# facebookresearch/theseus

Hardware: NVIDIA H100
Metric: LM iterations/sec on batched SE3 pose-graph (2500 poses, global batch 2048 over N GPUs, LM + block-sparse Cholesky, fp64) (higher is better)
Workload: dtype f64

## Files before the change

### theseus_b200/csrc/thb_front.cu

```cuda
#include <stdlib.h>

#include "thb_common.cuh"

namespace thb {

__device__ __forceinline__ void record_first_failure(int* info, int pos) {
  int old = 0;
  while (true) {
    const int prev = atomicCAS(info, old, pos);
    if (prev == old || (prev != 0 && prev <= pos)) return;
    old = prev;
  }
}

#ifdef THB_SIMT_EMU
#define THB_PDL_TRIGGER() do { } while (0)
#define THB_PDL_WAIT() do { } while (0)
#define FRONT_LAUNCH(K, grid, block, smem, cs, arg) K<<<grid, block, smem, cs>>>(arg)
#else
#define THB_PDL_TRIGGER() asm volatile("griddepcontrol.launch_dependents;" ::: "memory")
#define THB_PDL_WAIT() asm volatile("griddepcontrol.wait;" ::: "memory")
#define FRONT_LAUNCH(K, grid, block, smem, cs, arg) thb::front_launch_pdl(K, grid, block, smem, cs, arg)
static inline bool front_pdl_enabled() {
  static const bool on = [] { const char* e = getenv("THB_FRONT_PDL"); return e != nullptr && e[0] == '1'; }();
  return on;
}
template <typename A>
static inline void front_launch_pdl(void (*kernel)(A), dim3 grid, dim3 block, size_t smem, cudaStream_t cs, const A& arg) {
  cudaLaunchConfig_t cfg = {};
  cfg.gridDim = grid; cfg.blockDim = block; cfg.dynamicSmemBytes = smem; cfg.stream = cs;
  cudaLaunchAttribute at[1];
  at[0].id = cudaLaunchAttributeProgrammaticStreamSerialization;
  at[0].val.programmaticStreamSerializationAllowed = 1;
  cfg.attrs = at; cfg.numAttrs = front_pdl_enabled() ? 1 : 0;
  cudaLaunchKernelEx(&cfg, kernel, arg);
}
#endif

#ifdef THB_SIMT_EMU
__device__ inline void front_mma884(double& c0, double& c1, double a, double b) {
  const int lane = threadIdx.x & 31, lr = lane >> 2, lc = lane & 3;
  for (int k = 0; k < 4; k++) {
    const double av = __shfl_sync(0xffffffffu, a, lr * 4 + k);
    const double b0 = __shfl_sync(0xffffffffu, b, (2 * lc) * 4 + k);
    const double b1 = __shfl_sync(0xffffffffu, b, (2 * lc + 1) * 4 + k);
    c0 += av * b0;
    c1 += av * b1;
  }
}
#else
__device__ __forceinline__ void front_mma884(double& c0, double& c1, double a, double b) {
  asm volatile("mma.sync.aligned.m8n8k4.row.col.f64.f64.f64.f64 {%0,%1}, {%2}, {%3}, {%0,%1};\n" : "+d"(c0), "+d"(c1) : "d"(a), "d"(b));
}
#endif

__host__ __device__ __forceinline__ int front_pad_ld(int x) { return ((x + 11) / 16) * 16 + 4; }

struct FrontArgs {
  thb_front_plan p;
  int s0;
  int64_t B;
  double* factor;
  const double* alpha;
  const double* beta;
  double* arena_cur;
  const double* arena_child;
  int32_t* info;
  int prefetch;
  const double* ata;
  int64_t ata_stride;
  const double* rhs;
  double* work;
  double* v_cur;
  const double* v_child;
};

__device__ __forceinline__ double front_panel_in(const FrontArgs& a, const double* Lg, int64_t poff, int64_t item, int64_t e) {
  if (a.ata == nullptr) return Lg[e];
  const int32_t m = a.p.pmap[poff + e];
  return m >= 0 ? a.ata[item * a.ata_stride + m] : 0.0;
}

template <typename T>
__device__ __forceinline__ T front_ldg(const T* p) {
#ifdef THB_SIMT_EMU
  return *p;
#else
  return __ldg(p);
#endif
}


constexpr int FRONT_WD_LD = 20;
#ifndef FRONT_PL
#define FRONT_PL 4
#endif
constexpr int FRONT_MAX_CHILDREN = 8;

__host__ __device__ __forceinline__ int64_t front_smem_doubles(int w, int b, int nchildren) {
  const int b16 = (b + 15) & ~15, w8 = (w + 7) & ~7;
  return (int64_t)(w8 + b16 + 8) * front_pad_ld(w8) + 8 * FRONT_WD_LD + 3 * FRONT_MAX_CHILDREN
         + ((int64_t)nchildren * (w + b) + 1) / 2 + 2;
}

__device__ __forceinline__ int front_leaf8(double* __restrict__ T, int ld, double* __restrict__ Wd, int lane) {
  const int ln = lane < 8 ? lane : 0;
  double row[8];
#pragma unroll
  for (int q = 0; q < 8; q++) row[q] = T[ln * ld + q];
  int fail = 0;
  double invd = 0.0;
#pragma unroll
  for (int c = 0; c < 8; c++) {
    const double d = __shfl_sync(0xffffffffu, row[c], c);
    if (!(d > 0.0) && fail == 0) fail = c + 1;
    double inv = rsqrt(d);
    inv = inv * (1.5 - 0.5 * d * inv * inv);
    const double sq = d * inv;
    if (lane == c) invd = inv;
    const double lrc = (lane == c) ? sq : row[c] * inv;
    row[c] = lrc;
#pragma unroll
    for (int q = c + 1; q < 8; q++) {
      const double lqc = __shfl_sync(0xffffffffu, lrc, q);
      row[q] -= lrc * lqc;
    }
  }
  if (lane < 8) {
#pragma unroll
    for (int q = 0; q < 8; q++)
      if (q <= lane) T[lane * ld + q] = row[q];
  }
  double x[8];
#pragma unroll
  for (int rr = 0; rr < 8; rr++) {
    double sacc = (lane == rr) ? 1.0 : 0.0;
#pragma unroll
    for (int k = 0; k < rr; k++) {
      const double lrk = __shfl_sync(0xffffffffu, row[k], rr);
      sacc -= lrk * x[k];
    }
    x[rr] = sacc * __shfl_sync(0xffffffffu, invd, rr);
  }
  if (lane < 8) {
#pragma unroll
    for (int rr = 0; rr < 8; rr++) Wd[rr * FRONT_WD_LD + lane] = (rr >= lane) ? x[rr] : 0.0;
  }
  return fail;
}

__device__ __forceinline__ void front_diag_block(double* PN, int ldp, int jb, double* Wd, int lane, int w, int first, int32_t* info) {
  const int lr = lane >> 2, lc = lane & 3;
  double c0 = 0.0, c1 = 0.0;
  const double* Arow = PN + (8 * jb + lr) * ldp + lc;
  for (int k = 0; k < 8 * jb; k += 4) {
    const double av = Arow[k];
    front_mma884(c0, c1, av, av);
  }
  double* d = PN + (8 * jb + lr) * ldp + 8 * jb + 2 * lc;
  d[0] -= c0;
  d[1] -= c1;
  __syncwarp();
  const int fail = front_leaf8(PN + (8 * jb) * ldp + 8 * jb, ldp, Wd, lane);
  if (lane == 0 && fail != 0 && 8 * jb + fail <= w) record_first_failure(info, first + 8 * jb + fail);
}

template <bool TWO>
__device__ __forceinline__ void front_tile_column(double* PN, int ldp, int jb, int rt0, const double* Wd, int lane) {
  const int lr = lane >> 2, lc = lane & 3;
  double x00 = 0.0, x01 = 0.0, x10 = 0.0, x11 = 0.0;
  const double* A0 = PN + (8 * rt0 + lr) * ldp + lc;
  const double* Bj = PN + (8 * jb + lr) * ldp + lc;
  for (int k = 0; k < 8 * jb; k += 4) {
    const double bf = Bj[k];
    front_mma884(x00, x01, A0[k], bf);
    if (TWO) front_mma884(x10, x11, A0[8 * ldp + k], bf);
  }
  double* X0 = PN + (8 * rt0 + lr) * ldp + 8 * jb + 2 * lc;
  X0[0] -= x00; X0[1] -= x01;
  if (TWO) { X0[8 * ldp] -= x10; X0[8 * ldp + 1] -= x11; }
  __syncwarp();
  x00 = x01 = x10 = x11 = 0.0;
#pragma unroll
  for (int k = 0; k < 8; k += 4) {
    const double bf = Wd[lr * FRONT_WD_LD + k + lc];
    front_mma884(x00, x01, A0[8 * jb + k], bf);
    if (TWO) front_mma884(x10, x11, A0[8 * ldp + 8 * jb + k], bf);
  }
  __syncwarp();
  X0[0] = x00; X0[1] = x01;
  if (TWO) { X0[8 * ldp] = x10; X0[8 * ldp + 1] = x11; }
}

struct FrontChild {
  const double* src;
  int ldg, lo, hi, uoff;
};

__device__ __forceinline__ void front_panel_gather2(const FrontChild* ch, const int32_t* INV, int r, int nch, int q, const int* ii,
                                                    const int* jj, double (&x)[2][FRONT_PL]) {
#pragma unroll
  for (int c = 0; c < 2; c++) {
    int lo = r, hi = -1, ldg = 0;
    const double* src = nullptr;
    if (q + c < nch) { lo = ch[q + c].lo; hi = ch[q + c].hi; ldg = ch[q + c].ldg; src = ch[q + c].src; }
    const int32_t* inv = INV + (q + c) * r;
#pragma unroll
    for (int u = 0; u < FRONT_PL; u++) {
      x[c][u] = -0.0;
      if (ii[u] >= lo && jj[u] <= hi) {
        const int ci = inv[ii[u]], cj = inv[jj[u]];
        if (ci >= 0 && cj >= 0) x[c][u] = front_ldg(src + (int64_t)ci * ldg + cj);
      }
    }
  }
}

__device__ __forceinline__ int front_next_child(unsigned& mask) {
#ifdef THB_SIMT_EMU
  const int q = __builtin_ctz(mask);
#else
  const int q = __ffs(mask) - 1;
#endif
  mask &= mask - 1;
  return q;
}

__device__ __forceinline__ void front_tile_gather(const FrontChild& c, const int32_t* inv, int r, int li0, int lj0, double (&x)[2][2][2]) {
  int ci[2], cj[2][2];
#pragma unroll
  for (int mi = 0; mi < 2; mi++) ci[mi] = (li0 + 8 * mi < r) ? inv[li0 + 8 * mi] : -1;
#pragma unroll
  for (int ni = 0; ni < 2; ni++)
#pragma unroll
    for (int u = 0; u < 2; u++) cj[ni][u] = (lj0 + 8 * ni + u < r) ? inv[lj0 + 8 * ni + u] : -1;
#pragma unroll
  for (int mi = 0; mi < 2; mi++)
#pragma unroll
    for (int ni = 0; ni < 2; ni++)
#pragma unroll
      for (int u = 0; u < 2; u++)
        x[mi][ni][u] = (ci[mi] >= 0 && cj[ni][u] >= 0 && cj[ni][u] <= ci[mi]) ? front_ldg(c.src + (int64_t)ci[mi] * c.ldg + cj[ni][u]) : -0.0;
}

__device__ __forceinline__ double front_warp_trsv_lower(const double* T, int ld, double ui, int cw, int lane) {
  const double rd = lane < cw ? 1.0 / T[lane * ld + lane] : 0.0;
  for (int k = 0; k < cw; k++) {
    const double yk = __shfl_sync(0xffffffffu, ui * rd, k);
    if (lane == k) ui = yk;
    else if (lane > k && lane < cw) ui -= T[lane * ld + k] * yk;
  }
  return ui;
}

struct FrontRowsGlobal {
  static constexpr bool kInPanel = false;
  const double* L;
  int w;
  double* T;
  __device__ __forceinline__ const double* row(int i) const { return L + (int64_t)i * w; }
  __device__ __forceinline__ const double* diag(int k0, int cw, int tid, int nthreads, int* ld) const {
    for (int e = tid; e < cw * cw; e += nthreads) {
      const int i = e / cw, j = e - i * cw;
      T[i * 33 + j] = L[(int64_t)(k0 + i) * w + k0 + j];
    }
    *ld = 33;
    return T;
  }
};
struct FrontRowsPanel {
  static constexpr bool kInPanel = true;
  const double* PN;
  int ldp, w, shift;
  __device__ __forceinline__ const double* row(int i) const { return PN + (i < w ? i : i + shift) * ldp; }
  __device__ __forceinline__ const double* diag(int k0, int, int, int, int* ld) const {
    *ld = ldp;
    return PN + k0 * ldp + k0;
  }
};

template <int GROUP, bool WHOLE_CTA>
__device__ __forceinline__ void front_group_sync() {
#ifdef THB_SIMT_EMU
  static_assert(WHOLE_CTA, "the host emulation has no named barriers");
  __syncthreads();
#else
  if constexpr (WHOLE_CTA) __syncthreads();
  else asm volatile("bar.sync 1, %0;" ::"n"(GROUP) : "memory");
#endif
}

template <int GROUP, bool WHOLE_CTA, typename Rows>
__device__ __forceinline__ void front_forward_elim(const Rows& R, double* u, int us, int w, int r, int tid, int lane) {
  for (int k0 = 0; k0 < w; k0 += 32) {
    const int cw = min(32, w - k0);
    int ld;
    const double* T = R.diag(k0, cw, tid, GROUP, &ld);
    front_group_sync<GROUP, WHOLE_CTA>();
    if (tid < 32) {
      const double ui = front_warp_trsv_lower(T, ld, lane < cw ? u[(k0 + lane) * us] : 0.0, cw, lane);
      if (lane < cw) u[(k0 + lane) * us] = ui;
    }
    front_group_sync<GROUP, WHOLE_CTA>();
    for (int i = k0 + cw + tid; i < r; i += GROUP) {
      const double* row = R.row(i) + k0;
      double s = 0.0;
      if constexpr (Rows::kInPanel) {
        const int skew = (lane >> 2) & 3;
#pragma unroll 2
        for (int kk = 0; kk < cw + 3; kk++) {
          const int k = kk - skew;
          if ((unsigned)k < (unsigned)cw) s += row[k] * u[(k0 + k) * us];
        }
      } else {
        for (int k = 0; k < cw; k++) s += row[k] * u[(k0 + k) * us];
      }
      u[i * us] -= s;
    }
    front_group_sync<GROUP, WHOLE_CTA>();
  }
}

__device__ __forceinline__ void front_store_panel(double* __restrict__ Lg, const double* __restrict__ PN, int ldp, int w, int w8, int r, int tid,
                                                  int nthreads) {
  int i = tid / w, j = tid - i * w;
  const int di = nthreads / w, dj = nthreads - di * w;
  for (int e = tid; e < r * w; e += nthreads) {
    Lg[e] = (j > i) ? 0.0 : PN[(i < w ? i : i + (w8 - w)) * ldp + j];
    i += di; j += dj;
    if (j >= w) { j -= w; i++; }
  }
}

__device__ __forceinline__ void front_store_forward(const FrontArgs& a, const double* U, int ldp, int64_t item, int t, int f_first, int w, int b,
                                                    int tid, int nthreads) {
  for (int i = tid; i < w; i += nthreads) a.work[item * a.p.n + f_first + i] = U[i * ldp];
  double* ub = a.v_cur + item * a.p.varena_size + a.p.f_u_off[t];
  for (int i = tid; i < b; i += nthreads) ub[i] = U[(w + i) * ldp];
}

__host__ __device__ constexpr int front_elim_warps(int threads) { return threads >= 256 ? 4 : threads / 64; }

template <int THREADS>
__global__ void __launch_bounds__(THREADS, 1024 / THREADS) front_small_kernel(FrontArgs a) {
  extern __shared__ double sm[];
  const thb_front_plan& p = a.p;
  const int tid = threadIdx.x, lane = tid & 31, warp = tid >> 5;
  constexpr int NW = THREADS / 32;
  const int lr = lane >> 2, lc = lane & 3;
  const int64_t item = blockIdx.x;
  THB_PDL_TRIGGER();
  const int64_t* FD = p.fd + (int64_t)(a.s0 + blockIdx.y) * 8;
  const int t = (int)FD[0];
  const int w = (int)FD[1], b = (int)FD[2], r = w + b;
  const int f_first = (int)FD[3];
  const int64_t f_panel_off = FD[4];
  const int c_begin = (int)(FD[7] & 0xffffffffLL);
  const int nch = min((int)(FD[7] >> 32), FRONT_MAX_CHILDREN);
  const int b16 = (b + 15) & ~15, w8 = (w + 7) & ~7;
  const int ldp = front_pad_ld(w8);
  const int prow = w8 + b16 + 8;
  double* PN = sm;
  double* Wd = PN + prow * ldp;
  FrontChild* ch = reinterpret_cast<FrontChild*>(Wd + 8 * FRONT_WD_LD);
  int32_t* INV = reinterpret_cast<int32_t*>(Wd + 8 * FRONT_WD_LD + 3 * FRONT_MAX_CHILDREN);
  if (tid < nch) {
    const int64_t* PC = p.pc + (int64_t)(c_begin + tid) * 6;
    ch[tid].src = a.arena_child + item * p.arena_size + PC[0];
    ch[tid].ldg = (int)(PC[1] & 0xffffffffLL);
    ch[tid].lo = (int)PC[2];
    ch[tid].hi = (int)PC[3];
    ch[tid].uoff = (int)PC[5];
  }
  {
    int64_t ioff[FRONT_MAX_CHILDREN];
#pragma unroll
    for (int q = 0; q < FRONT_MAX_CHILDREN; q++) ioff[q] = q < nch ? p.pc[(int64_t)(c_begin + q) * 6 + 4] : 0;
    for (int l = tid; l < r; l += THREADS) {
      int32_t iv[FRONT_MAX_CHILDREN];
#pragma unroll
      for (int q = 0; q < FRONT_MAX_CHILDREN; q++) iv[q] = q < nch ? front_ldg(p.c_inv + ioff[q] + l) : 0;
#pragma unroll
      for (int q = 0; q < FRONT_MAX_CHILDREN; q++)
        if (q < nch) INV[q * r + l] = iv[q];
    }
  }
  for (int e = tid; e < prow * ldp; e += THREADS) sm[e] = 0.0;
  int* next_tile = reinterpret_cast<int*>(Wd + 8);
  if (tid == 0) *next_tile = 0;
  THB_PDL_WAIT();
#ifndef THB_SIMT_EMU
  if (a.rhs != nullptr) {
    for (int i = tid; i < w; i += THREADS) asm volatile("prefetch.global.L2 [%0];\n" ::"l"(a.rhs + item * p.n + p.perm[f_first + i]));
    for (int q = 0; q < nch; q++) {
      const int64_t* PC = p.pc + (int64_t)(c_begin + q) * 6;
      const double* cu = a.v_child + item * p.varena_size + PC[5];
      for (int off = tid * 16; off < (int)(PC[1] >> 32); off += THREADS * 16) asm volatile("prefetch.global.L2 [%0];\n" ::"l"(cu + off));
    }
  }
  for (int q = 0; a.prefetch != 0 && q < nch; q++) {
    const int64_t* PC = p.pc + (int64_t)(c_begin + q) * 6;
    const double* csrc = a.arena_child + item * p.arena_size + PC[0];
    const int cld = (int)(PC[1] & 0xffffffffLL), cbc = (int)(PC[1] >> 32);
    for (int off = tid * 16; off < cbc * cld; off += THREADS * 16) {
      const int i = off / cld, j = off - i * cld;
      if (j <= i) asm volatile("prefetch.global.L2 [%0];\n" ::"l"(csrc + off));
    }
  }
#endif
  __syncthreads();
  if (tid < w8 - w) PN[(w + tid) * ldp + w + tid] = 1.0;
  double* Lg = a.factor + item * p.data_size + f_panel_off;
  {
    const double al = a.alpha != nullptr ? a.alpha[item] : 0.0;
    const double be = a.beta != nullptr ? a.beta[item] : 0.0;
    const int total = r * w;
    for (int e0 = tid; e0 < total; e0 += FRONT_PL * THREADS) {
      int ii[FRONT_PL], jj[FRONT_PL];
      double v[FRONT_PL];
#pragma unroll
      for (int u = 0; u < FRONT_PL; u++) {
        const int e = e0 + u * THREADS;
        ii[u] = e / w;
        jj[u] = e - ii[u] * w;
        if (e >= total || jj[u] > ii[u]) ii[u] = -1;
      }
      int32_t m[FRONT_PL];
#pragma unroll
      for (int u = 0; u < FRONT_PL; u++) m[u] = (a.ata != nullptr && ii[u] >= 0) ? front_ldg(p.pmap + f_panel_off + e0 + u * THREADS) : -1;
      double x[2][FRONT_PL];
      front_panel_gather2(ch, INV, r, nch, 0, ii, jj, x);
#pragma unroll
      for (int u = 0; u < FRONT_PL; u++) {
        if (a.ata != nullptr) v[u] = m[u] >= 0 ? front_ldg(a.ata + item * a.ata_stride + m[u]) : 0.0;
        else v[u] = ii[u] >= 0 ? Lg[e0 + u * THREADS] : 0.0;
      }
#pragma unroll
      for (int u = 0; u < FRONT_PL; u++)
        if (ii[u] >= 0 && ii[u] == jj[u]) v[u] = v[u] + (al * v[u] + be);
      for (int q = 0;;) {
#pragma unroll
        for (int u = 0; u < FRONT_PL; u++) v[u] = (v[u] + x[0][u]) + x[1][u];
        q += 2;
        if (q >= nch) break;
        front_panel_gather2(ch, INV, r, nch, q, ii, jj, x);
      }
#pragma unroll
      for (int u = 0; u < FRONT_PL; u++)
        if (ii[u] >= 0) PN[(ii[u] < w ? ii[u] : ii[u] + (w8 - w)) * ldp + jj[u]] = v[u];
    }
  }
  double* U = PN + w8;
  if (a.rhs != nullptr) {
    for (int i = tid; i < r; i += THREADS) {
      double v = i < w ? a.rhs[item * p.n + p.perm[f_first + i]] : 0.0;
      for (int q = 0; q < nch; q++) {
        if (i >= ch[q].lo && i <= ch[q].hi) {
          const int k = INV[q * r + i];
          if (k >= 0) v += a.v_child[item * p.varena_size + ch[q].uoff + k];
        }
      }
      U[i * ldp] = v;
    }
  }
  __syncthreads();
  const int nbk = w8 / 8, nrt = (w8 + b16) / 8;
  for (int jb = 0; jb < nbk; jb++) {
    if (warp == 0) front_diag_block(PN, ldp, jb, Wd, lane, w, f_first, a.info + item);
    __syncthreads();
    const int npair = (nrt - jb) / 2;
    for (int q = warp; q < npair; q += NW) front_tile_column<true>(PN, ldp, jb, jb + 1 + 2 * q, Wd, lane);
    __syncthreads();
  }
#ifdef THB_SIMT_EMU
  front_store_panel(Lg, PN, ldp, w, w8, r, tid, THREADS);
  if (a.rhs != nullptr) {
    front_forward_elim<THREADS, true>(FrontRowsPanel{PN, ldp, w, w8 - w}, U, ldp, w, r, tid, lane);
    front_store_forward(a, U, ldp, item, t, f_first, w, b, tid, THREADS);
  }
#else
  constexpr int NE = front_elim_warps(THREADS);
  if (a.rhs != nullptr && warp < NE) {
    front_forward_elim<32 * NE, false>(FrontRowsPanel{PN, ldp, w, w8 - w}, U, ldp, w, r, tid, lane);
    front_store_forward(a, U, ldp, item, t, f_first, w, b, tid, 32 * NE);
  } else {
    const int t0 = a.rhs != nullptr ? 32 * NE : 0;
    front_store_panel(Lg, PN, ldp, w, w8, r, tid - t0, THREADS - t0);
  }
#endif
  if (b == 0) return;
  double* dst = a.arena_cur + item * p.arena_size + FD[5];
  const int ldg_out = (int)FD[6];
  const double* P = PN + w8 * ldp;
  const int nmt = b16 / 16;
  for (;;) {
    int q = 0;
    if (lane == 0) q = atomicAdd(next_tile, 1);
    q = __shfl_sync(0xffffffffu, q, 0);
    int R = (int)((sqrtf(8.0f * (float)q + 1.0f) - 1.0f) * 0.5f);
    while ((R + 1) * (R + 2) / 2 <= q) R++;
    while (R * (R + 1) / 2 > q) R--;
    if (R >= nmt) break;
    const int ct = q - R * (R + 1) / 2;
    unsigned reach = 0;
    for (int qc = 0; qc < nch; qc++)
      if (w + 16 * R + 15 >= ch[qc].lo && w + 16 * ct <= ch[qc].hi) reach |= 1u << qc;
    double gch[2][2][2] = {{{-0.0, -0.0}, {-0.0, -0.0}}, {{-0.0, -0.0}, {-0.0, -0.0}}};
    const int li0 = w + 16 * R + lr, lj0 = w + 16 * ct + 2 * lc;
    if (reach != 0) {
      const int qc = front_next_child(reach);
      front_tile_gather(ch[qc], INV + qc * r, r, li0, lj0, gch);
    }
    const bool summed = reach != 0;
    for (bool first = true; reach != 0; first = false) {
      const int qc = front_next_child(reach);
      double x[2][2][2];
      front_tile_gather(ch[qc], INV + qc * r, r, li0, lj0, x);
#pragma unroll
      for (int mi = 0; mi < 2; mi++)
#pragma unroll
        for (int ni = 0; ni < 2; ni++)
#pragma unroll
          for (int u = 0; u < 2; u++) gch[mi][ni][u] = (first ? 0.0 + gch[mi][ni][u] : gch[mi][ni][u]) + x[mi][ni][u];
    }
    double acc[2][2][2] = {{{0.0, 0.0}, {0.0, 0.0}}, {{0.0, 0.0}, {0.0, 0.0}}};
    const double* Pa = P + (16 * R + lr) * ldp + lc;
    const double* Pb = P + (16 * ct + lr) * ldp + lc;
#pragma unroll 1
    for (int k8 = 0; k8 < w8; k8 += 8) {
#pragma unroll
      for (int k4 = k8; k4 < k8 + 8; k4 += 4) {
        const double a0 = Pa[k4], a1 = Pa[8 * ldp + k4];
        const double b0 = Pb[k4], b1 = Pb[8 * ldp + k4];
        front_mma884(acc[0][0][0], acc[0][0][1], a0, b0);
        front_mma884(acc[0][1][0], acc[0][1][1], a0, b1);
        front_mma884(acc[1][0][0], acc[1][0][1], a1, b0);
        front_mma884(acc[1][1][0], acc[1][1][1], a1, b1);
      }
    }
    if (!summed) {
#pragma unroll
      for (int mi = 0; mi < 2; mi++)
#pragma unroll
        for (int ni = 0; ni < 2; ni++)
#pragma unroll
          for (int u = 0; u < 2; u++) gch[mi][ni][u] = 0.0 + gch[mi][ni][u];
    }
#pragma unroll
    for (int mi = 0; mi < 2; mi++)
#pragma unroll
      for (int ni = 0; ni < 2; ni++)
#pragma unroll
        for (int u = 0; u < 2; u++) acc[mi][ni][u] = gch[mi][ni][u] - acc[mi][ni][u];
#pragma unroll
    for (int mi = 0; mi < 2; mi++) {
      const int i = 16 * R + 8 * mi + lr;
      if (i < b) {
        double* drow = dst + (int64_t)i * ldg_out;
#pragma unroll
        for (int ni = 0; ni < 2; ni++)
#pragma unroll
          for (int u = 0; u < 2; u++) {
            const int jj = 16 * ct + 8 * ni + 2 * lc + u;
            if (jj <= i) drow[jj] = acc[mi][ni][u];
          }
      }
    }
  }
}

constexpr int ASM_ROWS = 16, ASM_THREADS = 256;

__device__ __forceinline__ int front_map_big(int l, int w, int wpad) { return l < w ? l : wpad + (l - w); }

__global__ void __launch_bounds__(ASM_THREADS, 4) front_assemble_kernel(FrontArgs a, int t) {
  extern __shared__ double sm[];
  const thb_front_plan& p = a.p;
  const int tid = threadIdx.x;
  const int64_t item = blockIdx.x;
  const int w = p.f_w[t], b = p.f_b[t], r = w + b, wpad = p.f_wpad[t], np = p.f_np[t];
  const int R0 = blockIdx.y * ASM_ROWS;
  const int nc = min(np, 128 * (R0 / 128 + 1));
  const int c_first = p.child_ptr[t], n_children = p.child_ptr[t + 1] - c_first;
  if (n_children <= FRONT_MAX_CHILDREN) {
    const double* Lgg = a.factor + item * p.data_size + p.f_panel_off[t];
    const double alg = a.alpha != nullptr ? a.alpha[item] : 0.0;
    const double beg = a.beta != nullptr ? a.beta[item] : 0.0;
    double* Fg = a.arena_cur + item * p.arena_size + p.f_fr_off[t] + (int64_t)R0 * np;
    __shared__ const double* s_src[FRONT_MAX_CHILDREN];
    __shared__ const int32_t* s_inv[FRONT_MAX_CHILDREN];
    __shared__ int s_ld[FRONT_MAX_CHILDREN];
    if (tid < n_children) {
      const int c = p.child_list[c_first + tid];
      s_src[tid] = a.arena_child + item * p.arena_size + p.f_cb_off[c];
      s_inv[tid] = p.c_inv + p.c_inv_ptr[c];
      s_ld[tid] = p.f_cb_ld[c];
    }
    __syncthreads();
    const int64_t poff = p.f_panel_off[t];
    const int total = ASM_ROWS * nc;
    auto gather2 = [&](int q, const int (&li)[4], const int (&lj)[4], double (&x)[2][4]) {
      int ci[2][4], cj[2][4];
#pragma unroll
      for (int c = 0; c < 2; c++) {
        const int32_t* inv = q + c < n_children ? s_inv[q + c] : nullptr;
#pragma unroll
        for (int u = 0; u < 4; u++) {
          ci[c][u] = (inv != nullptr && li[u] >= 0) ? front_ldg(inv + li[u]) : -1;
          cj[c][u] = (inv != nullptr && li[u] >= 0) ? front_ldg(inv + lj[u]) : -1;
        }
      }
#pragma unroll
      for (int c = 0; c < 2; c++) {
        const double* src = q + c < n_children ? s_src[q + c] : nullptr;
        const int ldg = q + c < n_children ? s_ld[q + c] : 0;
#pragma unroll
        for (int u = 0; u < 4; u++) x[c][u] = (ci[c][u] >= 0 && cj[c][u] >= 0) ? front_ldg(src + (int64_t)ci[c][u] * ldg + cj[c][u]) : -0.0;
      }
    };
    for (int e0 = tid; e0 < total; e0 += 4 * ASM_THREADS) {
      int li[4], lj[4];
      int pe[4];
      double v[4];
#pragma unroll
      for (int u = 0; u < 4; u++) {
        const int e = e0 + u * ASM_THREADS;
        const int rr = e / nc, fc = e - rr * nc;
        const int fr = R0 + rr;
        li[u] = fr < w ? fr : ((fr >= wpad && fr - wpad + w < r) ? fr - wpad + w : -1);
        lj[u] = fc < w ? fc : ((fc >= wpad && fc - wpad + w < r) ? fc - wpad + w : -1);
        v[u] = 0.0;
        pe[u] = -1;
        if (e >= total) {
          li[u] = lj[u] = -2;
        } else if (li[u] < 0 || lj[u] < 0) {
          v[u] = (fr == fc) ? 1.0 : 0.0;
          li[u] = -1;
        } else if (lj[u] > li[u]) {
          li[u] = -1;
        } else if (lj[u] < w) {
          pe[u] = li[u] * w + lj[u];
        }
      }
      int32_t m[4];
#pragma unroll
      for (int u = 0; u < 4; u++) m[u] = (a.ata != nullptr && pe[u] >= 0) ? front_ldg(p.pmap + poff + pe[u]) : -1;
      double x[2][4];
      gather2(0, li, lj, x);
#pragma unroll
      for (int u = 0; u < 4; u++) {
        if (a.ata != nullptr) { if (m[u] >= 0) v[u] = front_ldg(a.ata + item * a.ata_stride + m[u]); }
        else if (pe[u] >= 0) v[u] = Lgg[pe[u]];
      }
#pragma unroll
      for (int u = 0; u < 4; u++)
        if (li[u] >= 0 && li[u] == lj[u] && lj[u] < w) v[u] = v[u] + (alg * v[u] + beg);
      for (int q = 0;;) {
#pragma unroll
        for (int u = 0; u < 4; u++) v[u] = (v[u] + x[0][u]) + x[1][u];
        q += 2;
        if (q >= n_children) break;
        gather2(q, li, lj, x);
      }
#pragma unroll
      for (int u = 0; u < 4; u++) {
        const int e = e0 + u * ASM_THREADS;
        if (e < total) Fg[e + (int64_t)(e / nc) * (np - nc)] = v[u];
      }
    }
    return;
  }
  double* buf = sm;
  for (int e = tid; e < ASM_ROWS * nc; e += ASM_THREADS) buf[e] = 0.0;
  __syncthreads();
  const double* Lg = a.factor + item * p.data_size + p.f_panel_off[t];
  const double al = a.alpha != nullptr ? a.alpha[item] : 0.0;
  const double be = a.beta != nullptr ? a.beta[item] : 0.0;
  const int wlim = min(wpad, nc);
  for (int e = tid; e < ASM_ROWS * wlim; e += ASM_THREADS) {
    const int rr = e / wlim, j = e - rr * wlim;
    const int fr = R0 + rr;
    int i = -1;
    if (fr < w) i = fr;
    else if (fr >= wpad && fr - wpad + w < r) i = fr - wpad + w;
    if (i >= 0) {
      if (j < w && !(i < w && j > i)) {
        double v = front_panel_in(a, Lg, p.f_panel_off[t], item, (int64_t)i * w + j);
        if (i == j) v = v + (al * v + be);
        buf[rr * nc + j] = v;
      }
    } else if (j == fr) {
      buf[rr * nc + j] = 1.0;
    }
  }
  for (int rr = tid; rr < ASM_ROWS; rr += ASM_THREADS) {
    const int fr = R0 + rr;
    if (fr >= wpad + b) buf[rr * nc + fr] = 1.0;
  }
  __syncthreads();
  for (int ci = p.child_ptr[t]; ci < p.child_ptr[t + 1]; ci++) {
    const int c = p.child_list[ci];
    const int bc = p.f_b[c], ldg = p.f_cb_ld[c];
    const int32_t* rel = p.f_rel + p.rel_ptr[c];
    int lo = 0, hi = bc;
    while (lo < hi) { const int mid = (lo + hi) >> 1; if (front_map_big(rel[mid], w, wpad) < R0) lo = mid + 1; else hi = mid; }
    const int i0 = lo;
    hi = bc;
    while (lo < hi) { const int mid = (lo + hi) >> 1; if (front_map_big(rel[mid], w, wpad) < R0 + ASM_ROWS) lo = mid + 1; else hi = mid; }
    const int i1 = lo;
    if (i1 > i0) {
      const double* src = a.arena_child + item * p.arena_size + p.f_cb_off[c];
      for (int i = i0 + (tid >> 5); i < i1; i += ASM_THREADS / 32) {
        const int fr = front_map_big(rel[i], w, wpad) - R0;
        const double* srow = src + (int64_t)i * ldg;
        for (int j = tid & 31; j <= i; j += 32) buf[fr * nc + front_map_big(rel[j], w, wpad)] += srow[j];
      }
      __syncthreads();
    }
  }
  double* F = a.arena_cur + item * p.arena_size + p.f_fr_off[t] + (int64_t)R0 * np;
  for (int e = tid; e < ASM_ROWS * nc; e += ASM_THREADS) {
    const int rr = e / nc, c = e - rr * nc;
    F[(int64_t)rr * np + c] = buf[e];
  }
}

__global__ void __launch_bounds__(256) front_extract_kernel(FrontArgs a, int t) {
  const thb_front_plan& p = a.p;
  const int64_t item = blockIdx.x;
  const int w = p.f_w[t], b = p.f_b[t], r = w + b, wpad = p.f_wpad[t], np = p.f_np[t];
  const double* F = a.arena_cur + item * p.arena_size + p.f_fr_off[t];
  double* Lg = a.factor + item * p.data_size + p.f_panel_off[t];
  for (int e = blockIdx.y * blockDim.x + threadIdx.x; e < r * w; e += gridDim.y * blockDim.x) {
    const int i = e / w, j = e - i * w;
    const int fr = i < w ? i : wpad + (i - w);
    Lg[e] = (i < w && j > i) ? 0.0 : F[(int64_t)fr * np + j];
  }
}

struct FrontSolveArgs {
  thb_front_plan p;
  int s0;
  int64_t B;
  const double* factor;
  const double* rhs;
  double* x;
  double* work;
  double* v_cur;
  const double* v_child;
  int stage_doubles;
};

__device__ __forceinline__ double front_warp_trsv_upper(const double* T, double ti, int cw, int lane) {
  const double rd = lane < cw ? 1.0 / T[lane * 33 + lane] : 0.0;
  for (int k = cw - 1; k >= 0; k--) {
    const double xk = __shfl_sync(0xffffffffu, ti * rd, k);
    if (lane == k) ti = xk;
    else if (lane < k) ti -= T[k * 33 + lane] * xk;
  }
  return ti;
}

template <int THREADS>
__global__ void __launch_bounds__(THREADS) front_forward_kernel(FrontSolveArgs a) {
  extern __shared__ double sm[];
  const thb_front_plan& p = a.p;
  const int tid = threadIdx.x, lane = tid & 31;
  const int64_t item = blockIdx.x;
  THB_PDL_TRIGGER();
  const int64_t* FD = p.fd + (int64_t)(a.s0 + blockIdx.y) * 8;
  const int t = (int)FD[0];
  const int w = (int)FD[1], b = (int)FD[2], r = w + b, first = (int)FD[3];
  THB_PDL_WAIT();
  double* u = sm;
  double* T = sm + ((r + 1) & ~1);
  const double* Lg = a.factor + item * p.data_size + FD[4];
  if (r * w <= a.stage_doubles) {
    double* Ls = T + 32 * 33 + 1 + (THREADS & ~1) + 2;
    for (int e = tid; e < r * w; e += THREADS) Ls[e] = Lg[e];
    Lg = Ls;
  }
  {
    const int c0 = (int)(FD[7] & 0xffffffffLL), nchild = (int)(FD[7] >> 32);
    for (int i = tid; i < r; i += THREADS) {
      double v = i < w ? a.rhs[item * p.n + p.perm[first + i]] : 0.0;
      for (int q = 0; q < nchild; q++) {
        const int64_t* PC = p.pc + (int64_t)(c0 + q) * 6;
        if (i >= (int)PC[2] && i <= (int)PC[3]) {
          const int k = p.c_inv[PC[4] + i];
          if (k >= 0) v += a.v_child[item * p.varena_size + PC[5] + k];
        }
      }
      u[i] = v;
    }
  }
  __syncthreads();
  front_forward_elim<THREADS, true>(FrontRowsGlobal{Lg, w, T}, u, 1, w, r, tid, lane);
  for (int i = tid; i < w; i += THREADS) a.work[item * p.n + first + i] = u[i];
  if (b > 0) {
    double* ub = a.v_cur + item * p.varena_size + p.f_u_off[t];
    for (int i = tid; i < b; i += THREADS) ub[i] = u[w + i];
  }
}

template <int THREADS>
__global__ void __launch_bounds__(THREADS) front_backward_kernel(FrontSolveArgs a) {
  extern __shared__ double sm[];
  const thb_front_plan& p = a.p;
  const int tid = threadIdx.x, lane = tid & 31, warp = tid >> 5;
  const int64_t item = blockIdx.x;
  THB_PDL_TRIGGER();
  const int64_t* FD = p.fd + (int64_t)(a.s0 + blockIdx.y) * 8;
  const int t = (int)FD[0];
  const int w = (int)FD[1], b = (int)FD[2], r = w + b, first = (int)FD[3];
  THB_PDL_WAIT();
  double* xf = sm;
  double* T = sm + ((r + 1) & ~1);
  double* part = T + 32 * 33 + 1;
  const double* Lg = a.factor + item * p.data_size + FD[4];
  if (r * w <= a.stage_doubles) {
    double* Ls = T + 32 * 33 + 1 + (THREADS & ~1) + 2;
    for (int e = tid; e < r * w; e += THREADS) Ls[e] = Lg[e];
    Lg = Ls;
  }
  double* wk = a.work + item * p.n;
  const int32_t* rows = p.f_rows + p.rows_ptr[t];
  for (int i = tid; i < r; i += THREADS) xf[i] = i < w ? wk[first + i] : wk[rows[i - w]];
  __syncthreads();
  const int nchunk = (w + 31) / 32;
  for (int ch = nchunk - 1; ch >= 0; ch--) {
    const int k0 = ch * 32, cw = min(32, w - k0);
    const int RG = THREADS / cw;
    const int kk = tid % cw, rg = tid / cw;
    for (int e = tid; e < cw * cw; e += THREADS) {
      const int i = e / cw, j = e - i * cw;
      T[i * 33 + j] = Lg[(int64_t)(k0 + i) * w + k0 + j];
    }
    double acc = 0.0;
    if (rg < RG) {
      const double* col = Lg + k0 + kk;
      int i = k0 + cw + rg;
      for (; i + 3 * RG < r; i += 4 * RG) {
        const double l0 = col[(int64_t)i * w], l1 = col[(int64_t)(i + RG) * w], l2 = col[(int64_t)(i + 2 * RG) * w],
                     l3 = col[(int64_t)(i + 3 * RG) * w];
        acc += l0 * xf[i];
        acc += l1 * xf[i + RG];
        acc += l2 * xf[i + 2 * RG];
        acc += l3 * xf[i + 3 * RG];
      }
      for (; i < r; i += RG) acc += col[(int64_t)i * w] * xf[i];
    }
    part[tid] = acc;
    __syncthreads();
    if (warp == 0) {
      double tk = 0.0;
      if (lane < cw) {
        tk = xf[k0 + lane];
        for (int g = 0; g < RG; g++) tk -= part[g * cw + lane];
      }
      tk = front_warp_trsv_upper(T, tk, cw, lane);
      if (lane < cw) xf[k0 + lane] = tk;
    }
    __syncthreads();
  }
  for (int i = tid; i < w; i += THREADS) {
    const double v = xf[i];
    wk[first + i] = v;
    a.x[item * p.n + p.perm[first + i]] = v;
  }
}

static inline int front_threads_of_class(int cls) { return cls == 0 ? 64 : (cls == 1 ? 128 : 256); }

template <typename K>
static inline int front_set_smem(K kernel, size_t bytes, size_t* cache) {
  if (bytes > *cache) {
    cudaError_t e = cudaFuncSetAttribute(kernel, cudaFuncAttributeMaxDynamicSharedMemorySize, (int)bytes);
    if (e != cudaSuccess) return (int)e;
    *cache = bytes;
  }
  return 0;
}

static int front_solve_launch(const thb_front_plan* p, const int64_t* L, int pass, const double* factor, const double* rhs, double* x,
                              double* work, double* varena, int64_t B, cudaStream_t cs) {
  static size_t fw_set[3] = {0, 0, 0}, bw_set[3] = {0, 0, 0};
  static const int64_t stage_cap = [] { const char* e = getenv("THB_SOLVE_STAGE"); return e != nullptr ? (int64_t)atoll(e) : (int64_t)0; }();
  const int depth = (int)L[0], cls = (int)L[1], begin = (int)L[2], count = (int)L[3];
  FrontSolveArgs a;
  a.p = *p; a.s0 = begin; a.B = B; a.factor = factor; a.rhs = rhs; a.x = x; a.work = work;
  a.v_cur = varena != nullptr ? varena + (int64_t)(depth & 1) * B * p->varena_size : nullptr;
  a.v_child = varena != nullptr ? varena + (int64_t)((depth + 1) & 1) * B * p->varena_size : nullptr;
  const int kc = cls > 2 ? 2 : cls;
  const int threads = front_threads_of_class(kc);
  const int64_t r_max = L[5];
  const int64_t stage = (cls < 3 && L[6] > 0) ? (L[6] < stage_cap ? L[6] : stage_cap) : 0;
  a.stage_doubles = (int)stage;
  const size_t smem = (size_t)(((r_max + 1) & ~1LL) + 32 * 33 + 1 + threads + 2 + stage + 2) * 8;
  const dim3 grid((unsigned)B, (unsigned)count);
  if (pass == 0) {
    if (kc == 0) { int rc = front_set_smem(front_forward_kernel<64>, smem, &fw_set[0]); if (rc) return rc;
                   FRONT_LAUNCH(front_forward_kernel<64>, grid, 64, smem, cs, a); }
    else if (kc == 1) { int rc = front_set_smem(front_forward_kernel<128>, smem, &fw_set[1]); if (rc) return rc;
                        FRONT_LAUNCH(front_forward_kernel<128>, grid, 128, smem, cs, a); }
    else { int rc = front_set_smem(front_forward_kernel<256>, smem, &fw_set[2]); if (rc) return rc;
           FRONT_LAUNCH(front_forward_kernel<256>, grid, 256, smem, cs, a); }
  } else {
    if (kc == 0) { int rc = front_set_smem(front_backward_kernel<64>, smem, &bw_set[0]); if (rc) return rc;
                   FRONT_LAUNCH(front_backward_kernel<64>, grid, 64, smem, cs, a); }
    else if (kc == 1) { int rc = front_set_smem(front_backward_kernel<128>, smem, &bw_set[1]); if (rc) return rc;
                        FRONT_LAUNCH(front_backward_kernel<128>, grid, 128, smem, cs, a); }
    else { int rc = front_set_smem(front_backward_kernel<256>, smem, &bw_set[2]); if (rc) return rc;
           FRONT_LAUNCH(front_backward_kernel<256>, grid, 256, smem, cs, a); }
  }
  THB_CHECK_LAUNCH();
  return THB_OK;
}

static int front_factor(const thb_front_plan* p, const int64_t* launches, int64_t num_launches, double* factor, const double* ata,
                        int64_t ata_stride, const double* alpha, const double* beta, double* arena, void* dense_ws, int64_t dense_ws_bytes,
                        int32_t* info, const double* rhs, double* work, double* varena, int64_t B, thb_stream_t stream) {
  if (p == nullptr || launches == nullptr || factor == nullptr || arena == nullptr || info == nullptr || B < 0) return THB_ERR_BAD_ARG;
  if (B == 0 || p->S == 0) return THB_OK;
  if (B > 65535LL * 32768LL) return THB_ERR_UNSUPPORTED;
  cudaStream_t cs = thb_cs(stream);
  THB_CUDA(cudaMemsetAsync(info, 0, (size_t)B * 4, cs));
  static size_t smem_set[5] = {0, 0, 0, 0, 0}, asm_set = 0;
  static const int thr_cls[2] = {[] { const char* e = getenv("THB_FRONT_T0"); const int v = e ? atoi(e) : 64; return (v == 128 || v == 256) ? v : 64; }(),
                                 [] { const char* e = getenv("THB_FRONT_T1"); const int v = e ? atoi(e) : 128; return v == 256 ? 256 : 128; }()};
  static int front_prefetch_flag = -1;
  if (front_prefetch_flag < 0) {
    const char* e = getenv("THB_FRONT_PREFETCH");
    front_prefetch_flag = (e != nullptr && e[0] == '1') ? 1 : 0;
  }
  static const int fuse_max = [] { const char* e = getenv("THB_FRONT_FUSE_MAX"); return e != nullptr ? atoi(e) : 1024; }();
  for (int64_t l = 0; l < num_launches; l++) {
    const int64_t* L = launches + l * THB_FRONT_LAUNCH_COLS;
    const int depth = (int)L[0], cls = (int)L[1], begin = (int)L[2], count = (int)L[3];
    FrontArgs a;
    a.p = *p; a.s0 = begin; a.B = B; a.factor = factor; a.alpha = alpha; a.beta = beta; a.info = info;
    a.ata = (ata != nullptr && p->pmap != nullptr) ? ata : nullptr; a.ata_stride = ata_stride;
    a.prefetch = front_prefetch_flag;
    a.arena_cur = arena + (int64_t)(depth & 1) * B * p->arena_size;
    a.arena_child = arena + (int64_t)((depth + 1) & 1) * B * p->arena_size;
    a.rhs = rhs; a.work = work;
    a.v_cur = rhs != nullptr ? varena + (int64_t)(depth & 1) * B * p->varena_size : nullptr;
    a.v_child = rhs != nullptr ? varena + (int64_t)((depth + 1) & 1) * B * p->varena_size : nullptr;
    if (cls < 3) {
      const size_t smem = (size_t)L[4];
#ifndef THB_SIMT_EMU
      if (smem > 227 * 1024) return THB_ERR_UNSUPPORTED;
#endif
      const dim3 grid((unsigned)B, (unsigned)count);
      if (count > 65535) return THB_ERR_UNSUPPORTED;
      const int threads = (cls == 0 && thr_cls[0] == 64) ? 64
                          : ((cls == 0 && thr_cls[0] == 128) || (cls == 1 && thr_cls[1] == 128)) ? 128
                          : (cls <= 1 || smem <= 56 * 1024) ? 256 : (smem <= 113 * 1024 ? 512 : 1024);
      const bool fused = rhs != nullptr && threads <= fuse_max;
      if (!fused) a.rhs = nullptr;
      if (threads == 64) {
        int rc = front_set_smem(front_small_kernel<64>, smem, &smem_set[0]); if (rc) return rc;
        FRONT_LAUNCH(front_small_kernel<64>, grid, 64, smem, cs, a);
      } else if (threads == 128) {
        int rc = front_set_smem(front_small_kernel<128>, smem, &smem_set[1]); if (rc) return rc;
        FRONT_LAUNCH(front_small_kernel<128>, grid, 128, smem, cs, a);
      } else if (threads == 256) {
        int rc = front_set_smem(front_small_kernel<256>, smem, &smem_set[2]); if (rc) return rc;
        FRONT_LAUNCH(front_small_kernel<256>, grid, 256, smem, cs, a);
      } else if (threads == 512) {
        int rc = front_set_smem(front_small_kernel<512>, smem, &smem_set[3]); if (rc) return rc;
        FRONT_LAUNCH(front_small_kernel<512>, grid, 512, smem, cs, a);
      } else {
        int rc = front_set_smem(front_small_kernel<1024>, smem, &smem_set[4]); if (rc) return rc;
        FRONT_LAUNCH(front_small_kernel<1024>, grid, 1024, smem, cs, a);
      }
      THB_CHECK_LAUNCH();
      if (rhs != nullptr && !fused) {
        const int rc = front_solve_launch(p, L, 0, factor, rhs, nullptr, work, varena, B, cs);
        if (rc != THB_OK) return rc;
      }
    } else {
      const int64_t np = L[5], nb_piv = L[6], fr_off = L[7], first = L[8];
      const int t = (int)L[9];
#ifdef THB_SIMT_EMU
      (void)np; (void)nb_piv; (void)fr_off; (void)first; (void)t; (void)dense_ws; (void)dense_ws_bytes; (void)asm_set;
      return THB_ERR_UNSUPPORTED;
#else
      if (dense_ws == nullptr || np % 128 != 0 || np > 8192) return THB_ERR_BAD_ARG;
      const size_t smem = (size_t)ASM_ROWS * np * 8;
      int rc = front_set_smem(front_assemble_kernel, smem, &asm_set); if (rc) return rc;
      front_assemble_kernel<<<dim3((unsigned)B, (unsigned)(np / ASM_ROWS)), ASM_THREADS, smem, cs>>>(a, t);
      THB_CHECK_LAUNCH();
      rc = thb_potrf_partial_inplace_f64(a.arena_cur + fr_off, p->arena_size, np, (int32_t)nb_piv, (int32_t)L[10], (int32_t)(nb_piv * 64 + L[11]),
                                         (int32_t)first, info, B, dense_ws, dense_ws_bytes, stream);
      if (rc != THB_OK) return rc;
      front_extract_kernel<<<dim3((unsigned)B, 8), 256, 0, cs>>>(a, t);
      THB_CHECK_LAUNCH();
      if (rhs != nullptr) {
        rc = front_solve_launch(p, L, 0, factor, rhs, nullptr, work, varena, B, cs);
        if (rc != THB_OK) return rc;
      }
#endif
    }
  }
  return THB_OK;
}

}

extern "C" {

int64_t thb_front_small_smem_bytes(int32_t w, int32_t b, int32_t nchildren) { return thb::front_smem_doubles(w, b, nchildren) * 8; }

int thb_front_factor_f64(const thb_front_plan* p, const int64_t* launches, int64_t num_launches, double* factor, const double* ata,
                         int64_t ata_stride, const double* alpha, const double* beta, double* arena, void* dense_ws, int64_t dense_ws_bytes,
                         int32_t* info, int64_t B, thb_stream_t stream) {
  return thb::front_factor(p, launches, num_launches, factor, ata, ata_stride, alpha, beta, arena, dense_ws, dense_ws_bytes, info, nullptr,
                           nullptr, nullptr, B, stream);
}

int thb_front_factor_forward_f64(const thb_front_plan* p, const int64_t* launches, int64_t num_launches, double* factor, const double* ata,
                                 int64_t ata_stride, const double* alpha, const double* beta, double* arena, void* dense_ws,
                                 int64_t dense_ws_bytes, int32_t* info, const double* rhs, double* work, double* varena, int64_t B,
                                 thb_stream_t stream) {
  if (rhs == nullptr || work == nullptr || varena == nullptr) return THB_ERR_BAD_ARG;
  return thb::front_factor(p, launches, num_launches, factor, ata, ata_stride, alpha, beta, arena, dense_ws, dense_ws_bytes, info, rhs, work,
                           varena, B, stream);
}

int thb_front_solve_f64(const thb_front_plan* p, const int64_t* launches, int64_t num_launches, const double* factor, const double* rhs,
                        double* x, double* work, double* varena, int64_t B, thb_stream_t stream) {
  if (p == nullptr || launches == nullptr || factor == nullptr || rhs == nullptr || x == nullptr || work == nullptr || varena == nullptr ||
      B < 0)
    return THB_ERR_BAD_ARG;
  if (B == 0 || p->S == 0) return THB_OK;
  const int rc = thb_front_forward_f64(p, launches, num_launches, factor, rhs, work, varena, B, stream);
  if (rc != THB_OK) return rc;
  return thb_front_backward_f64(p, launches, num_launches, factor, x, work, B, stream);
}

int thb_front_forward_f64(const thb_front_plan* p, const int64_t* launches, int64_t num_launches, const double* factor, const double* rhs,
                          double* work, double* varena, int64_t B, thb_stream_t stream) {
  if (p == nullptr || launches == nullptr || factor == nullptr || rhs == nullptr || work == nullptr || varena == nullptr || B < 0)
    return THB_ERR_BAD_ARG;
  if (B == 0 || p->S == 0) return THB_OK;
  cudaStream_t cs = thb_cs(stream);
  for (int64_t q = 0; q < num_launches; q++) {
    const int rc = thb::front_solve_launch(p, launches + q * THB_FRONT_LAUNCH_COLS, 0, factor, rhs, nullptr, work, varena, B, cs);
    if (rc != THB_OK) return rc;
  }
  return THB_OK;
}

int thb_front_backward_f64(const thb_front_plan* p, const int64_t* launches, int64_t num_launches, const double* factor, double* x,
                           double* work, int64_t B, thb_stream_t stream) {
  if (p == nullptr || launches == nullptr || factor == nullptr || x == nullptr || work == nullptr || B < 0) return THB_ERR_BAD_ARG;
  if (B == 0 || p->S == 0) return THB_OK;
  cudaStream_t cs = thb_cs(stream);
  for (int64_t q = num_launches - 1; q >= 0; q--) {
    const int rc = thb::front_solve_launch(p, launches + q * THB_FRONT_LAUNCH_COLS, 1, factor, nullptr, x, work, nullptr, B, cs);
    if (rc != THB_OK) return rc;
  }
  return THB_OK;
}

}
```

Baseline: 5.644.

## Overlap diagonal-block factorization with off-diagonal assembly and defer row-tile updates

```diff
diff --git a/theseus_b200/csrc/thb_front.cu b/theseus_b200/csrc/thb_front.cu
--- a/theseus_b200/csrc/thb_front.cu
+++ b/theseus_b200/csrc/thb_front.cu
@@ -103,7 +103,7 @@
          + ((int64_t)nchildren * (w + b) + 1) / 2 + 2;
 }
 
-__device__ __forceinline__ int front_leaf8(double* __restrict__ T, int ld, double* __restrict__ Wd, int lane) {
+__device__ __forceinline__ int front_leaf8(double* __restrict__ T, int ld, double* __restrict__ Wd, int ldw, int lane) {
   const int ln = lane < 8 ? lane : 0;
   double row[8];
 #pragma unroll
@@ -144,12 +144,28 @@
   }
   if (lane < 8) {
 #pragma unroll
-    for (int rr = 0; rr < 8; rr++) Wd[rr * FRONT_WD_LD + lane] = (rr >= lane) ? x[rr] : 0.0;
+    for (int rr = 0; rr < 8; rr++) Wd[rr * ldw + lane] = (rr >= lane) ? x[rr] : 0.0;
   }
   return fail;
 }
 
-__device__ __forceinline__ void front_diag_block(double* PN, int ldp, int jb, double* Wd, int lane, int w, int first, int32_t* info) {
+__device__ __forceinline__ double* front_winv(double* PN, int ldp, double* Wd, int jb, int nbk, int* ldw) {
+  const bool last = jb + 1 == nbk;
+  *ldw = last ? FRONT_WD_LD : ldp;
+  return last ? Wd : PN + (8 * jb) * ldp + 8 * jb + 8;
+}
+
+__device__ __forceinline__ int front_laneid() {
+#ifdef THB_SIMT_EMU
+  return threadIdx.x & 31;
+#else
+  int l;
+  asm volatile("mov.u32 %0, %%laneid;" : "=r"(l));
+  return l;
+#endif
+}
+
+__device__ __forceinline__ void front_diag_block(double* PN, int ldp, int jb, double* Wd, int ldw, int lane, int w, int first, int32_t* info) {
   const int lr = lane >> 2, lc = lane & 3;
   double c0 = 0.0, c1 = 0.0;
   const double* Arow = PN + (8 * jb + lr) * ldp + lc;
@@ -161,12 +177,12 @@
   d[0] -= c0;
   d[1] -= c1;
   __syncwarp();
-  const int fail = front_leaf8(PN + (8 * jb) * ldp + 8 * jb, ldp, Wd, lane);
+  const int fail = front_leaf8(PN + (8 * jb) * ldp + 8 * jb, ldp, Wd, ldw, lane);
   if (lane == 0 && fail != 0 && 8 * jb + fail <= w) record_first_failure(info, first + 8 * jb + fail);
 }
 
 template <bool TWO>
-__device__ __forceinline__ void front_tile_column(double* PN, int ldp, int jb, int rt0, const double* Wd, int lane) {
+__device__ __forceinline__ void front_tile_column(double* PN, int ldp, int jb, int rt0, const double* Wd, int ldw, int lane) {
   const int lr = lane >> 2, lc = lane & 3;
   double x00 = 0.0, x01 = 0.0, x10 = 0.0, x11 = 0.0;
   const double* A0 = PN + (8 * rt0 + lr) * ldp + lc;
@@ -183,7 +199,7 @@
   x00 = x01 = x10 = x11 = 0.0;
 #pragma unroll
   for (int k = 0; k < 8; k += 4) {
-    const double bf = Wd[lr * FRONT_WD_LD + k + lc];
+    const double bf = Wd[lr * ldw + k + lc];
     front_mma884(x00, x01, A0[8 * jb + k], bf);
     if (TWO) front_mma884(x10, x11, A0[8 * ldp + 8 * jb + k], bf);
   }
@@ -410,30 +426,29 @@
 #endif
   __syncthreads();
   if (tid < w8 - w) PN[(w + tid) * ldp + w + tid] = 1.0;
-  double* Lg = a.factor + item * p.data_size + f_panel_off;
-  {
-    const double al = a.alpha != nullptr ? a.alpha[item] : 0.0;
-    const double be = a.beta != nullptr ? a.beta[item] : 0.0;
-    const int total = r * w;
-    for (int e0 = tid; e0 < total; e0 += FRONT_PL * THREADS) {
+  const double al = a.alpha != nullptr ? a.alpha[item] : 0.0;
+  const double be = a.beta != nullptr ? a.beta[item] : 0.0;
+  auto assemble = [&](int e_begin, int e_end, int t, int nt) {
+    const double* Lg = a.factor + item * p.data_size + f_panel_off;
+    for (int e0 = e_begin + t; e0 < e_end; e0 += FRONT_PL * nt) {
       int ii[FRONT_PL], jj[FRONT_PL];
       double v[FRONT_PL];
 #pragma unroll
       for (int u = 0; u < FRONT_PL; u++) {
-        const int e = e0 + u * THREADS;
+        const int e = e0 + u * nt;
         ii[u] = e / w;
         jj[u] = e - ii[u] * w;
-        if (e >= total || jj[u] > ii[u]) ii[u] = -1;
+        if (e >= e_end || jj[u] > ii[u]) ii[u] = -1;
       }
       int32_t m[FRONT_PL];
 #pragma unroll
-      for (int u = 0; u < FRONT_PL; u++) m[u] = (a.ata != nullptr && ii[u] >= 0) ? front_ldg(p.pmap + f_panel_off + e0 + u * THREADS) : -1;
+      for (int u = 0; u < FRONT_PL; u++) m[u] = (a.ata != nullptr && ii[u] >= 0) ? front_ldg(p.pmap + f_panel_off + e0 + u * nt) : -1;
       double x[2][FRONT_PL];
       front_panel_gather2(ch, INV, r, nch, 0, ii, jj, x);
 #pragma unroll
       for (int u = 0; u < FRONT_PL; u++) {
         if (a.ata != nullptr) v[u] = m[u] >= 0 ? front_ldg(a.ata + item * a.ata_stride + m[u]) : 0.0;
-        else v[u] = ii[u] >= 0 ? Lg[e0 + u * THREADS] : 0.0;
+        else v[u] = ii[u] >= 0 ? Lg[e0 + u * nt] : 0.0;
       }
 #pragma unroll
       for (int u = 0; u < FRONT_PL; u++)
@@ -449,29 +464,49 @@
       for (int u = 0; u < FRONT_PL; u++)
         if (ii[u] >= 0) PN[(ii[u] < w ? ii[u] : ii[u] + (w8 - w)) * ldp + jj[u]] = v[u];
     }
-  }
+  };
+  assemble(0, w * w, tid, THREADS);
+  __syncthreads();
+  const int nbk = w8 / 8;
   double* U = PN + w8;
-  if (a.rhs != nullptr) {
-    for (int i = tid; i < r; i += THREADS) {
-      double v = i < w ? a.rhs[item * p.n + p.perm[f_first + i]] : 0.0;
-      for (int q = 0; q < nch; q++) {
-        if (i >= ch[q].lo && i <= ch[q].hi) {
-          const int k = INV[q * r + i];
-          if (k >= 0) v += a.v_child[item * p.varena_size + ch[q].uoff + k];
+  if (warp == 0) {
+    for (int jb = 0; jb < nbk; jb++) {
+      int ldw;
+      double* W = front_winv(PN, ldp, Wd, jb, nbk, &ldw);
+      __syncwarp();
+      front_diag_block(PN, ldp, jb, W, ldw, front_laneid(), w, f_first, a.info + item);
+      for (int rt = jb + 1; rt < nbk; rt += 2) {
+        __syncwarp();
+        if (rt + 1 < nbk) front_tile_column<true>(PN, ldp, jb, rt, W, ldw, lane);
+        else front_tile_column<false>(PN, ldp, jb, rt, W, ldw, lane);
+      }
+    }
+  } else {
+    assemble(w * w, r * w, tid - 32, THREADS - 32);
+    if (a.rhs != nullptr) {
+      for (int i = tid - 32; i < r; i += THREADS - 32) {
+        double v = i < w ? a.rhs[item * p.n + p.perm[f_first + i]] : 0.0;
+        for (int q = 0; q < nch; q++) {
+          if (i >= ch[q].lo && i <= ch[q].hi) {
+            const int k = INV[q * r + i];
+            if (k >= 0) v += a.v_child[item * p.varena_size + ch[q].uoff + k];
+          }
         }
-      }
-      U[i * ldp] = v;
+        U[i * ldp] = v;
+      }
     }
   }
   __syncthreads();
-  const int nbk = w8 / 8, nrt = (w8 + b16) / 8;
-  for (int jb = 0; jb < nbk; jb++) {
-    if (warp == 0) front_diag_block(PN, ldp, jb, Wd, lane, w, f_first, a.info + item);
-    __syncthreads();
-    const int npair = (nrt - jb) / 2;
-    for (int q = warp; q < npair; q += NW) front_tile_column<true>(PN, ldp, jb, jb + 1 + 2 * q, Wd, lane);
-    __syncthreads();
-  }
+  for (int q = warp; q < b16 / 16; q += NW) {
+    for (int jb = 0; jb < nbk; jb++) {
+      int ldw;
+      const double* W = front_winv(PN, ldp, Wd, jb, nbk, &ldw);
+      __syncwarp();
+      front_tile_column<true>(PN, ldp, jb, nbk + 2 * q, W, ldw, lane);
+    }
+  }
+  __syncthreads();
+  double* Lg = a.factor + item * p.data_size + FD[4];
 #ifdef THB_SIMT_EMU
   front_store_panel(Lg, PN, ldp, w, w8, r, tid, THREADS);
   if (a.rhs != nullptr) {
```

Result: faster. 5.744 (median of 6 runs) (+1.8%).
